# Senpai-sama06/real-time-audio-visual-zooming

Measured on AMD Instinct MI355X. Metric: beamformed TF-bins/sec (2-ch, 1024-pt STFT) + SIR dB delta vs reference, higher is better.
Workload: dtype f32; 1 GPU; configs[1]: B=256 utterances/GPU, 2 interferers, oracle IBM, 1024-pt STFT hop 512 @16 kHz, 4.0 s utterances; batch_per_gpu=256, global_batch=256, samples=64000, n_fft=1024, hop=512, parallelism=utterance-sharded x1, RCCL metric all-reduce only, input_batches=2, tf_bins_per_utt=64638, mask=ibm, postfilter=ibm, normalize=peak

## Files before the change

real-time-audio-visual-zooming_amd/csrc/avz_chain_exact.hpp:

```cpp
#pragma once
#include "avz_chain_common.hpp"
#include "avz_ibm_exact.hpp"

namespace avz {
__device__ __forceinline__ int pick(uint32_t packed, int i) {
  return (int)(signed char)(packed >> (8 * i));
}
template <int N>
struct XLds {
  using C = KCfg<N>;
  using X = XGeo<N>;
  static constexpr int FR = 4;
  static constexpr int MP = N / 2 + 4;
  static constexpr int MIC_BYTES = FR / C::FPW * C::WAVE_BYTES;
  static constexpr int MAG_OFF = (4 * X::SCRATCH > MIC_BYTES) ? 4 * X::SCRATCH : MIC_BYTES;
  static constexpr int TWL_OFF = MAG_OFF + 2 * FR * MP * 4;
  static constexpr int WIN_OFF = TWL_OFF + (N / 2) * 16;
  static constexpr int SLOT_OFF = WIN_OFF + N * 4;
  static constexpr int SCAN_OFF = SLOT_OFF + FR * 32;
  static constexpr int SCAN_INTS = 256;
  static constexpr int WL = 32;
  static constexpr int WL_OFF = SCAN_OFF + 256 * 4;
  static constexpr int CTL_OFF = WL_OFF + WL * 16;
  static constexpr int END = CTL_OFF + 32;
  static_assert(C::FPW == 2 && END <= CGeo<N>::SLOT_LDS, "exact phase LDS");
};

struct XSlot {
  int unit, f, e, b, L, c, flags, pad;
};
__device__ __forceinline__ XSlot slot_u(const XSlot* sl, int g) {
  const XSlot v = sl[g];
  XSlot s;
  s.unit = __builtin_amdgcn_readfirstlane(v.unit);
  s.f = __builtin_amdgcn_readfirstlane(v.f);
  s.e = 0;
  s.b = __builtin_amdgcn_readfirstlane(v.b);
  s.L = __builtin_amdgcn_readfirstlane(v.L);
  s.c = __builtin_amdgcn_readfirstlane(v.c);
  s.flags = __builtin_amdgcn_readfirstlane(v.flags);
  s.pad = 0;
  return s;
}

template <int N, bool PER_BIN>
__device__ __forceinline__ void exact_round(KArgs& A, unsigned char* lds, const XSlot* sl, int ns,
                                            Acc32 (&pacc)[CGeo<N>::BPT + 1],
                                            uint32_t (&pbits)[CGeo<N>::BPT + 1]) {
  using C = KCfg<N>;
  using G = CGeo<N>;
  using X = XGeo<N>;
  using XL = XLds<N>;
  constexpr int NT = G::NT, H = G::H, F = G::F, BPT = G::BPT, PPL = C::PPL, MP = XL::MP;
  const int tid = threadIdx.x, lane = tid & 63;
  const int wave = __builtin_amdgcn_readfirstlane(tid >> 6);
  float* const mag = reinterpret_cast<float*>(lds + XL::MAG_OFF);
  const cd* const twl = reinterpret_cast<const cd*>(lds + XL::TWL_OFF);
  const float* const win = reinterpret_cast<const float*>(lds + XL::WIN_OFF);
  cd* const buf = reinterpret_cast<cd*>(lds + wave * X::SCRATCH);
  AVZ_STAMP_DECL();
  AVZ_STAMP_INIT();
  AVZ_XT_LAP_BEGIN(xr_prev);
  int lane_o = lane;
  opaque_i(lane_o);
  const int ga = wave >> 1, gb = (wave >> 1) + 2;
  const float* const refp = (wave & 1) ? A.ref_int : A.ref_tgt;
  float xa[N / 64], xb[N / 64];
  if (ga < ns) {
    const XSlot s = slot_u(sl, ga);
    ref_frame_load<N>(make_rsrc(refp + (long long)s.b * A.ref_stride, s.L),
                      (s.c * kChunk + s.f) * H - N / 2, lane_o, xa);
  }
  if (gb < ns) {
    const XSlot s = slot_u(sl, gb);
    ref_frame_load<N>(make_rsrc(refp + (long long)s.b * A.ref_stride, s.L),
                      (s.c * kChunk + s.f) * H - N / 2, lane_o, xb);
  }
  if (ga < ns) ref_spectrum_exact<N>(xa, twl, win, buf, mag + (2 * ga + (wave & 1)) * MP, lane_o);
  AVZ_STAMP(4);
  AVZ_XT_LAP(8, xr_prev);
  cf v[PPL];
  LaneMap<N> lm;
  lm.init(lane_o);
  const int gm = C::FPW * wave + lm.grp;
  if (wave < XL::FR / C::FPW) {
    const XSlot s = slot_u(sl, 0);
    const float* mixb = A.mix + (long long)s.b * A.mix_stride;
    const rsrc_t r_m0 = make_rsrc(mixb, s.L), r_m1 = make_rsrc(mixb + A.ch_stride, s.L);
    const bool on = gm < ns;
    const int fm = sl[on ? gm : 0].f;
    const int s0 = (s.c * kChunk + fm) * H - N / 2 + lm.in0;
#pragma unroll
    for (int r = 0; r < PPL; ++r) {
      v[r].x = on ? bload(r_m0, s0 + C::IN_STRIDE * r) : 0.0f;
      v[r].y = on ? bload(r_m1, s0 + C::IN_STRIDE * r) : 0.0f;
    }
  }
  if (gb < ns) {
    int lane_b = lane;
    opaque_i(lane_b);
    ref_spectrum_exact<N>(xb, twl, win, buf, mag + (2 * gb + (wave & 1)) * MP, lane_b);
  }
  AVZ_STAMP(5);
  lds_barrier();
  AVZ_STAMP(6);
  AVZ_XT_LAP(9, xr_prev);
  if (wave < XL::FR / C::FPW) {
    WinCoef<N> wc;
    wc.init(lm);
    cf* const spec = slot_ptr<N>(lds, gm);
    if constexpr (N == 1024) {
      Fft1024x2 f;
      f.l = lm.out0;
      window_apply(v, wc.a0, wc.ac, wc.as);
      f.forward(v, spec, reinterpret_cast<const cf*>(lds + G::TW_OFF));
      static_for<0, 32>([&](auto k) { spec[lm.out0 + 32 * k] = v[k]; });
    } else {
      Fft512x2 f;
      f.init(lane_o);
      window_fft<N>(v, wc, f, spec, lm);
    }
  }
  AVZ_STAMP(7);
  lds_barrier();
  AVZ_STAMP(8);
  AVZ_XT_LAP(10, xr_prev);
  unsigned long long n_exact = 0;
  for (int g = 0; g < ns; ++g) {
    const XSlot s = slot_u(sl, g);
    const cf* Zm = slot_ptr<N>(lds, g);
    auto put = [&](int j, int k, const Acc32& a, bool dfr, bool noise) {
      if (dfr) {
        pacc[j].c00 += a.c00;
        pacc[j].c11 += a.c11;
        pacc[j].c01r += a.c01r;
        pacc[j].c01i += a.c01i;
        pacc[j].cm += a.cm;
        pbits[j] |= (noise ? 1u : 0u) << s.f;
      }
    };
#pragma unroll
    for (int j = 0; j < BPT; ++j) {
      const int kb = tid + j * NT;
      const int kp = (N - kb) & (N - 1);
      const bool dfr =
          PER_BIN ? ((A.xdfr[(long long)s.unit * F + kb] >> s.f) & 1u)
                  : ((s.flags & 1) &&
                     ((A.xunc[((long long)s.unit * kChunk + s.f) * 32 + (kb & 31)] >> (kb >> 5)) & 1u));
      Acc32 a;
      a.zero();
      bool noise = false;
      if (dfr) {
        noise = mag[(2 * g + 1) * MP + kb] > mag[(2 * g) * MP + kb];
        cf x0, x1;
        split_pair2(Zm[kb], Zm[kp], x0, x1);
        a.add_sel(x0, x1, noise);
        a.cm = noise ? 1.0f : 0.0f;
        n_exact += 1;
      }
      put(j, kb, a, dfr, noise);
    }
    if (tid == NT - 1) {
      const bool dfr = (s.flags >> 1) & 1;
      Acc32 a;
      a.zero();
      bool noise = false;
      if (dfr) {
        noise = mag[(2 * g + 1) * MP + N / 2] > mag[(2 * g) * MP + N / 2];
        cf y0, y1;
        split_pair2(Zm[N / 2], Zm[N / 2], y0, y1);
        const float wn = noise ? 1.0f : 0.0f;
        a.add(y0, y1, wn, wn);
        n_exact += 1;
      }
      put(BPT, N / 2, a, dfr, noise);
    }
  }
  if (A.xstat && n_exact) atomicAdd(A.xstat + 1, n_exact);
  AVZ_STAMP(9);
  lds_barrier();
  AVZ_STAMP(10);
  AVZ_XT_LAP(11, xr_prev);
}

constexpr int kSparseMax = 12;

constexpr uint32_t kXOpen = 0x80000000u;
constexpr int kXRound = 2;
struct XPieces {
  uint32_t sp;
  int n_sp, nr, npr, n;
};
__device__ __forceinline__ XPieces x_pieces(uint32_t pend, uint32_t big) {
  XPieces q;
  q.sp = pend & ~big;
  q.n_sp = q.sp ? 1 : 0;
  q.nr = (__popc(big) + kXRound - 1) / kXRound;
  q.npr = min(q.nr, kXPieces - q.n_sp);
  q.n = q.n_sp + q.npr;
  return q;
}
__device__ __forceinline__ bool x_has_piece(uint32_t v) {
  return (v & kXOpen) && (v & 0xffffu) < ((v >> 16) & 0xffu);
}

template <int N>
__device__ __forceinline__ void exact_sparse(KArgs& A, unsigned char* lds, int b, int L, int c,
                                             const int* items, int n,
                                             Acc32 (&pacc)[CGeo<N>::BPT + 1],
                                             uint32_t (&pbits)[CGeo<N>::BPT + 1]) {
  using G = CGeo<N>;
  using XL = XLds<N>;
  constexpr int H = N / 2, NT = G::NT, BPT = G::BPT;
  const int tid = threadIdx.x, lane = tid & 63;
  const int wave = __builtin_amdgcn_readfirstlane(tid >> 6);
  const cd* const twl = reinterpret_cast<const cd*>(lds + XL::TWL_OFF);
  const float* const win = reinterpret_cast<const float*>(lds + XL::WIN_OFF);
  float* const res = reinterpret_cast<float*>(lds);
  const rsrc_t rt = make_rsrc(A.ref_tgt + (long long)b * A.ref_stride, L);
  const rsrc_t ri = make_rsrc(A.ref_int + (long long)b * A.ref_stride, L);
  const float* mixb = A.mix + (long long)b * A.mix_stride;
  const rsrc_t rm0 = make_rsrc(mixb, L), rm1 = make_rsrc(mixb + A.ch_stride, L);
  for (int it = wave; it < n; it += NT / 64) {
    const int item = __builtin_amdgcn_readfirstlane(items[it]);
    const int f = item >> 16, k = item & 0xffff;
    const int s0 = (c * kChunk + f) * H - N / 2;
    float st[N / 64], si[N / 64], sm0[N / 64], sm1[N / 64];
#pragma unroll
    for (int r = 0; r < N / 64; ++r) {
      const int m = lane + 64 * r;
      st[r] = bload(rt, s0 + m);
      si[r] = bload(ri, s0 + m);
      sm0[r] = bload(rm0, s0 + m);
      sm1[r] = bload(rm1, s0 + m);
    }
    double tr = 0.0, ti = 0.0, ir = 0.0, ii = 0.0, ac = 0.0, bs = 0.0, as = 0.0, bc = 0.0;
#pragma unroll
    for (int r = 0; r < N / 64; ++r) {
      const int m = lane + 64 * r;
      const double w = (double)win[m];
      const double xt = w * (double)st[r], xi = w * (double)si[r];
      const double a = w * (double)sm0[r], bb = w * (double)sm1[r];
      const cd tw = xtw_at<N>(twl, (k * m) & (N - 1));
      tr = fma(xt, tw.x, tr);
      ti = fma(xt, tw.y, ti);
      ir = fma(xi, tw.x, ir);
      ii = fma(xi, tw.y, ii);
      ac = fma(a, tw.x, ac);
      bs = fma(bb, tw.y, bs);
      as = fma(a, tw.y, as);
      bc = fma(bb, tw.x, bc);
    }
#pragma unroll
    for (int o = 32; o > 0; o >>= 1) {
      tr += __shfl_xor(tr, o, 64);
      ti += __shfl_xor(ti, o, 64);
      ir += __shfl_xor(ir, o, 64);
      ii += __shfl_xor(ii, o, 64);
      ac += __shfl_xor(ac, o, 64);
      bs += __shfl_xor(bs, o, 64);
      as += __shfl_xor(as, o, 64);
      bc += __shfl_xor(bc, o, 64);
    }
    if (lane == 0) {
      const bool noise = np_abs_c64((float)ir, (float)ii) > np_abs_c64((float)tr, (float)ti);
      constexpr double sc = 2.0 / N;
      const cf zk = {(float)(sc * (ac - bs)), (float)(sc * (as + bc))};
      const cf zp = {(float)(sc * (ac + bs)), (float)(sc * (bc - as))};
      Acc32 t;
      t.zero();
      cf x0, x1;
      split_pair2(zk, zp, x0, x1);
      if (k == N / 2) {
        const float wn = noise ? 1.0f : 0.0f;
        t.add(x0, x1, wn, wn);
      } else {
        t.add_sel(x0, x1, noise);
        t.cm = noise ? 1.0f : 0.0f;
      }
      float* q = res + 6 * it;
      q[0] = noise ? 1.0f : 0.0f;
      q[1] = t.c00;
      q[2] = t.c11;
      q[3] = t.c01r;
      q[4] = t.c01i;
      q[5] = t.cm;
    }
  }
  __syncthreads();
  for (int it = 0; it < n; ++it) {
    const int item = items[it];
    const int f = item >> 16, k = item & 0xffff;
    const int j = k == N / 2 ? BPT : k / NT;
    if (k == N / 2 ? tid == NT - 1 : (k % NT) == tid) {
      const float* q = res + 6 * it;
#pragma unroll
      for (int jj = 0; jj <= BPT; ++jj) {
        if (jj != j) continue;
        pacc[jj].c00 += q[1];
        pacc[jj].c11 += q[2];
        pacc[jj].c01r += q[3];
        pacc[jj].c01i += q[4];
        pacc[jj].cm += q[5];
        pbits[jj] |= (q[0] != 0.0f ? 1u : 0u) << f;
      }
    }
  }
  if (A.xstat && tid == 0) atomicAdd(A.xstat + 1, (unsigned long long)n);
  __syncthreads();
}

template <int N, bool PER_BIN, class CA>
__device__ __forceinline__ void exact_set_slot(CA& A, XSlot* sl, int g, int u, int f, int gx,
                                               int n_items, int n_whole, int P) {
  constexpr int F = N / 2 + 1;
  XSlot s;
  s.unit = u;
  s.f = f;
  s.e = -1;
  unit_item<F>(A, u, gx, n_items, n_whole, P, s.b, s.c);
  s.L = utt_len(A, s.b);
  const uint4 r = reinterpret_cast<const uint4*>(A.xpend)[u];
  s.flags = (PER_BIN ? 0 : (int)((r.y >> f) & 1u)) | (int)(((r.z >> f) & 1u) << 1);
  s.pad = 0;
  sl[g] = s;
}

template <int N, bool PER_BIN>
__device__ __forceinline__ void exact_unit(KArgs& A, unsigned char* lds, int u, int gx, int n_items,
                                           int n_whole, int P) {
  using G = CGeo<N>;
  using XL = XLds<N>;
  constexpr int F = N / 2 + 1, NT = G::NT, BPT = G::BPT, FR = XL::FR;
  const int tid = threadIdx.x;
  XSlot* const sl = reinterpret_cast<XSlot*>(lds + XL::SLOT_OFF);
  const uint4 rec = reinterpret_cast<const uint4*>(A.xpend)[u];
  const uint32_t pend = rec.x;
  if (pend == 0u || rec.w != 0u) return;
  int b, c;
  float* const Pt = unit_item<F>(A, u, gx, n_items, n_whole, P, b, c);
  if (A.xstat && tid == 0) atomicAdd(A.xstat, (unsigned long long)__popc(pend));
  Acc32 pacc[BPT + 1];
  uint32_t pbits[BPT + 1];
#pragma unroll
  for (int j = 0; j <= BPT; ++j) {
    const int kk = j < BPT ? tid + j * NT : N / 2;
    pbits[j] = 0u;
    if (j < BPT || tid == NT - 1) {
      pacc[j].c00 = Pt[0 * F + kk];
      pacc[j].c11 = Pt[1 * F + kk];
      pacc[j].c01r = Pt[2 * F + kk];
      pacc[j].c01i = Pt[3 * F + kk];
      pacc[j].cm = Pt[4 * F + kk];
    } else {
      pacc[j].zero();
    }
  }
  uint32_t rest = pend;
  if constexpr (!PER_BIN) {
    int* const items = reinterpret_cast<int*>(lds + XL::SCAN_OFF);
    int* const ctl = reinterpret_cast<int*>(lds + XL::CTL_OFF);
    uint32_t* const wsm = reinterpret_cast<uint32_t*>(lds + 16384);
    const uint32_t has_words = reinterpret_cast<const uint4*>(A.xpend)[u].y;
#pragma unroll
    for (int i = 0; i < kChunk / (G::NT / 32); ++i) {
      const int f = (tid >> 5) + (G::NT / 32) * i;
      if ((pend >> f) & 1u)
        wsm[f * 32 + (tid & 31)] =
            ((has_words >> f) & 1u) ? A.xunc[((long long)u * kChunk + f) * 32 + (tid & 31)] : 0u;
    }
    __syncthreads();
    if (tid < 64) {
      const uint32_t nyq = reinterpret_cast<const uint4*>(A.xpend)[u].z;
      int base = 0;
      uint32_t sparse = 0u;
      for (uint32_t todo = pend; todo != 0u; todo &= todo - 1u) {
        const int f = __builtin_ctz(todo);
        const uint32_t w = tid < 32 ? wsm[f * 32 + tid] : 0u;
        int inc = __popc(w);
#pragma unroll
        for (int o = 1; o < 32; o <<= 1) {
          const int y = __shfl_up(inc, o, 64);
          if ((tid & 63) >= o) inc += y;
        }
        const int tot = __shfl(inc, 31, 64), ny = (nyq >> f) & 1u;
        if (tot + ny <= kSparseMax && base + tot + ny <= XL::SCAN_INTS) {
          int at = base + inc - __popc(w);
          for (uint32_t x = w; x != 0u; x &= x - 1u) items[at++] = (f << 16) | (tid + 32 * __builtin_ctz(x));
          if (ny && tid == 0) items[base + tot] = (f << 16) | (N / 2);
          base += tot + ny;
          sparse |= 1u << f;
        }
      }
      if (tid == 0) {
        ctl[0] = base;
        ctl[1] = (int)sparse;
      }
    }
    __syncthreads();
    const int n_sp = ctl[0];
    rest &= ~(uint32_t)ctl[1];
    if (n_sp > 0) exact_sparse<N>(A, lds, b, utt_len(A, b), c, items, n_sp, pacc, pbits);
  }
  while (rest != 0u) {
    if (tid < FR) {
      uint32_t x = rest;
      for (int i = 0; i < tid && x; ++i) x &= x - 1u;
      if (x) exact_set_slot<N, PER_BIN>(A, sl, tid, u, __builtin_ctz(x), gx, n_items, n_whole, P);
    }
    const int ns = min(FR, __popc(rest));
    for (int i = 0; i < ns; ++i) rest &= rest - 1u;
    __syncthreads();
    exact_round<N, PER_BIN>(A, lds, sl, ns, pacc, pbits);
  }
  uint32_t* const MW = A.mwords + ((long long)b * A.nchunk + c) * F;
#pragma unroll
  for (int j = 0; j <= BPT; ++j) {
    const int kk = j < BPT ? tid + j * NT : N / 2;
    if (j < BPT || tid == NT - 1) {
      Pt[0 * F + kk] = pacc[j].c00;
      Pt[1 * F + kk] = pacc[j].c11;
      Pt[2 * F + kk] = pacc[j].c01r;
      Pt[3 * F + kk] = pacc[j].c01i;
      Pt[4 * F + kk] = pacc[j].cm;
      if (pbits[j]) atomicOr(MW + kk, pbits[j]);
    }
  }
}

template <int N>
__device__ __forceinline__ void exact_sparse_frames(KArgs& A, unsigned char* lds, int u, int b,
                                                    int c, uint32_t frames,
                                                    Acc32 (&pacc)[CGeo<N>::BPT + 1],
                                                    uint32_t (&pbits)[CGeo<N>::BPT + 1]) {
  using G = CGeo<N>;
  using XL = XLds<N>;
  const int tid = threadIdx.x;
  int* const items = reinterpret_cast<int*>(lds + XL::SCAN_OFF);
  int* const ctl = reinterpret_cast<int*>(lds + XL::CTL_OFF);
  uint32_t* const wsm = reinterpret_cast<uint32_t*>(lds + 16384);
  const uint4 rec = reinterpret_cast<const uint4*>(A.xpend)[u];
#pragma unroll
  for (int i = 0; i < kChunk / (G::NT / 32); ++i) {
    const int f = (tid >> 5) + (G::NT / 32) * i;
    if ((frames >> f) & 1u)
      wsm[f * 32 + (tid & 31)] =
          ((rec.y >> f) & 1u) ? A.xunc[((long long)u * kChunk + f) * 32 + (tid & 31)] : 0u;
  }
  __syncthreads();
  uint32_t todo = frames;
  while (todo != 0u) {
    if (tid < 64) {
      int base = 0;
      uint32_t took = 0u;
      for (uint32_t t = todo; t != 0u; t &= t - 1u) {
        const int f = __builtin_ctz(t);
        const uint32_t w = tid < 32 ? wsm[f * 32 + tid] : 0u;
        int inc = __popc(w);
#pragma unroll
        for (int o = 1; o < 32; o <<= 1) {
          const int y = __shfl_up(inc, o, 64);
          if ((tid & 63) >= o) inc += y;
        }
        const int tot = __shfl(inc, 31, 64), ny = (rec.z >> f) & 1u;
        if (base + tot + ny > XL::SCAN_INTS) break;
        int at = base + inc - __popc(w);
        for (uint32_t x = w; x != 0u; x &= x - 1u) items[at++] = (f << 16) | (tid + 32 * __builtin_ctz(x));
        if (ny && tid == 0) items[base + tot] = (f << 16) | (N / 2);
        base += tot + ny;
        took |= 1u << f;
      }
      if (tid == 0) {
        ctl[0] = base;
        ctl[1] = (int)took;
      }
    }
    __syncthreads();
    const int n = ctl[0];
    todo &= ~(uint32_t)ctl[1];
    exact_sparse<N>(A, lds, b, utt_len(A, b), c, items, n, pacc, pbits);
  }
}

template <int N, bool PER_BIN>
__device__ __forceinline__ void exact_piece(KArgs& A, unsigned char* lds, int u, int p, int gx,
                                            int n_items, int n_whole, int P) {
  using G = CGeo<N>;
  using XL = XLds<N>;
  constexpr int F = N / 2 + 1, NT = G::NT, BPT = G::BPT, FR = XL::FR;
  const int tid = threadIdx.x;
  XSlot* const sl = reinterpret_cast<XSlot*>(lds + XL::SLOT_OFF);
  int* const ctl = reinterpret_cast<int*>(lds + XL::CTL_OFF);
  const uint4 rec = reinterpret_cast<const uint4*>(A.xpend)[u];
  const XPieces q = x_pieces(rec.x, rec.w);
  int b, c;
  float* const Pt = unit_item<F>(A, u, gx, n_items, n_whole, P, b, c);
  Acc32 pacc[BPT + 1];
  uint32_t pbits[BPT + 1];
#pragma unroll
  for (int j = 0; j <= BPT; ++j) {
    pacc[j].zero();
    pbits[j] = 0u;
  }
  if (p < q.n_sp) {
    if (A.xstat && tid == 0) atomicAdd(A.xstat, (unsigned long long)__popc(q.sp));
    if constexpr (!PER_BIN) exact_sparse_frames<N>(A, lds, u, b, c, q.sp, pacc, pbits);
  } else {
    constexpr int R = kXRound;
    static_assert(R <= FR, "round frames");
    const int g = p - q.n_sp, r0 = g * q.nr / q.npr, r1 = (g + 1) * q.nr / q.npr;
    if (A.xstat && tid == 0)
      atomicAdd(A.xstat, (unsigned long long)(min(R * r1, __popc(rec.w)) - R * r0));
    const int L = utt_len(A, b);
    uint32_t rest = rec.w;
    for (int i = 0; i < r0 * R; ++i) rest &= rest - 1u;
    for (int r = r0; r < r1; ++r) {
      if (tid < R) {
        uint32_t x = rest;
        for (int i = 0; i < tid && x; ++i) x &= x - 1u;
        if (x) {
          const int f = __builtin_ctz(x);
          XSlot s;
          s.unit = u;
          s.f = f;
          s.e = -1;
          s.b = b;
          s.L = L;
          s.c = c;
          s.flags = (PER_BIN ? 0 : (int)((rec.y >> f) & 1u)) | (int)(((rec.z >> f) & 1u) << 1);
          s.pad = 0;
          sl[tid] = s;
        }
      }
      const int ns = min(R, __popc(rest));
      for (int i = 0; i < ns; ++i) rest &= rest - 1u;
      __syncthreads();
      exact_round<N, PER_BIN>(A, lds, sl, ns, pacc, pbits);
    }
  }
  uint32_t* const MW = A.mwords + ((long long)b * A.nchunk + c) * F;
  float* const R = A.xres + ((long long)u * kXPieces + p) * 5 * F;
#pragma unroll
  for (int j = 0; j <= BPT; ++j) {
    const int kk = j < BPT ? tid + j * NT : N / 2;
    if (j < BPT || tid == NT - 1) {
      if (pbits[j]) atomicOr(MW + kk, pbits[j]);
      if (q.n == 1) {
        Pt[0 * F + kk] = Pt[0 * F + kk] + pacc[j].c00;
        Pt[1 * F + kk] = Pt[1 * F + kk] + pacc[j].c11;
        Pt[2 * F + kk] = Pt[2 * F + kk] + pacc[j].c01r;
        Pt[3 * F + kk] = Pt[3 * F + kk] + pacc[j].c01i;
        Pt[4 * F + kk] = Pt[4 * F + kk] + pacc[j].cm;
      } else {
        R[0 * F + kk] = pacc[j].c00;
        R[1 * F + kk] = pacc[j].c11;
        R[2 * F + kk] = pacc[j].c01r;
        R[3 * F + kk] = pacc[j].c01i;
        R[4 * F + kk] = pacc[j].cm;
      }
    }
  }
#ifdef AVZ_XTRACE
  const unsigned long long tf = __builtin_amdgcn_s_memrealtime();
#endif
  __syncthreads();
  if (tid == 0) {
    bool last = true;
    if (q.n > 1) {
      __builtin_amdgcn_fence(__ATOMIC_RELEASE, "agent");
      const uint32_t arrived =
          __hip_atomic_fetch_add(A.xst + 2 * u + 1, 1u, __ATOMIC_RELAXED, __HIP_MEMORY_SCOPE_AGENT) + 1u;
      last = arrived == (uint32_t)q.n;
      if (last) __builtin_amdgcn_fence(__ATOMIC_ACQUIRE, "agent");
    }
    ctl[4] = last ? 1 : 0;
  }
  __syncthreads();
#ifdef AVZ_XTRACE
  const unsigned long long tm = __builtin_amdgcn_s_memrealtime();
  if (tid == 0 && g_stamps) g_stamps[blockIdx.x * 16 + 6] += tm - tf;
#endif
  if (ctl[4]) {
    if (q.n > 1) {
      const float* const R0 = A.xres + (long long)u * kXPieces * 5 * F;
      constexpr int M = (5 * F + NT - 1) / NT;
      float v[M];
#pragma unroll
      for (int m = 0; m < M; ++m) v[m] = tid + m * NT < 5 * F ? Pt[tid + m * NT] : 0.0f;
      for (int pp = 0; pp < q.n; ++pp) {
        float t[M];
#pragma unroll
        for (int m = 0; m < M; ++m)
          t[m] = tid + m * NT < 5 * F ? R0[(long long)pp * 5 * F + tid + m * NT] : 0.0f;
#pragma unroll
        for (int m = 0; m < M; ++m) v[m] += t[m];
      }
#pragma unroll
      for (int m = 0; m < M; ++m)
        if (tid + m * NT < 5 * F) Pt[tid + m * NT] = v[m];
    }
    if (tid == 0) {
      __hip_atomic_store(A.xst + 2 * u + 1, 0u, __ATOMIC_RELAXED, __HIP_MEMORY_SCOPE_AGENT);
      __hip_atomic_store(A.xst + 2 * u, 0u, __ATOMIC_RELAXED, __HIP_MEMORY_SCOPE_AGENT);
      __hip_atomic_fetch_and(A.xhint + (u >> 5), ~(1u << (u & 31)), __ATOMIC_RELAXED,
                             __HIP_MEMORY_SCOPE_AGENT);
    }
  }
  __syncthreads();
#ifdef AVZ_XTRACE
  if (tid == 0 && g_stamps) g_stamps[blockIdx.x * 16 + 7] += __builtin_amdgcn_s_memrealtime() - tm;
#endif
}

__device__ __forceinline__ int exact_claim(KArgs& A, int n_units, int* cand) {
  const int lane = threadIdx.x & 63;
  const int nw = (n_units + 31) >> 5;
  const int w_start = (int)(((long long)blockIdx.x * nw) / gridDim.x);
  for (;;) {
    int count = 0;
    for (int w0 = 0; w0 < nw && count < 64; w0 += 64) {
      const int wi = w0 + lane;
      int wid = w_start + wi;
      if (wid >= nw) wid -= nw;
      const uint32_t bits =
          wi < nw ? __hip_atomic_load(A.xhint + wid, __ATOMIC_RELAXED, __HIP_MEMORY_SCOPE_AGENT) : 0u;
      const int cnt = __popc(bits);
      int pre = cnt;
#pragma unroll
      for (int o = 1; o < 64; o <<= 1) {
        const int y = __shfl_up(pre, o, 64);
        if (lane >= o) pre += y;
      }
      const int tot = __shfl(pre, 63, 64);
      int pos = count + pre - cnt;
      for (uint32_t x = bits; x != 0u && pos < 64; x &= x - 1u) cand[pos++] = wid * 32 + __builtin_ctz(x);
      count += tot;
    }
    count = min(count, 64);
    if (count == 0) return -1;
    __builtin_amdgcn_fence(__ATOMIC_RELEASE, "wavefront");
    __builtin_amdgcn_wave_barrier();
    __builtin_amdgcn_fence(__ATOMIC_ACQUIRE, "wavefront");
    const int uid = lane < count ? cand[lane] : -1;
    const uint32_t v =
        uid >= 0 ? __hip_atomic_load(A.xst + 2 * uid, __ATOMIC_RELAXED, __HIP_MEMORY_SCOPE_AGENT) : 0u;
    const unsigned long long m = __ballot(x_has_piece(v));
    if (m == 0ull) return -1;
    int k = (int)(blockIdx.x % (unsigned)__popcll(m));
    unsigned long long mm = m;
    for (; k > 0; --k) mm &= mm - 1ull;
    const int src = __builtin_ctzll(mm);
    int res = -1;
    if (lane == src) {
      const uint32_t old =
          __hip_atomic_fetch_add(A.xst + 2 * uid, 1u, __ATOMIC_RELAXED, __HIP_MEMORY_SCOPE_AGENT);
      if (x_has_piece(old)) {
        __builtin_amdgcn_fence(__ATOMIC_ACQUIRE, "agent");
        res = (uid << 8) | (int)(old & 0xffu);
      }
    }
    res = __shfl(res, src, 64);
    if (res >= 0) return res;
    __builtin_amdgcn_wave_barrier();
  }
}

template <int N, int MASK, bool IRM, bool SPLIT, class TW>
__device__ __forceinline__ void ibm_exact_units(unsigned char* lds, int gx, int n_items) {
  KArgs& A = kernarg_chain_args();
  using G = CGeo<N>;
  using XL = XLds<N>;
  constexpr bool SHARE = N == 1024 && !std::is_same<TW, NoTw>::value;
  constexpr bool PER_BIN = !(N == 1024 && !IRM && SHARE);
  AVZ_XT(1, __builtin_amdgcn_s_memrealtime());
  if (A.ibm_cert <= 0.0f) return;
  const int tid = threadIdx.x;
  const int P = SPLIT && A.a_pieces > 1 ? A.a_pieces : 1;
  const int n_whole = P > 1 ? A.a_whole : n_items;
  __syncthreads();
  const uint32_t mine = *reinterpret_cast<const uint32_t*>(lds + G::MISC_OFF + 56);
  auto tables = [&]() {
    int t = threadIdx.x;
    opaque_i(t);
    xtab_fill<N>(A.xtw, A.xwin, reinterpret_cast<cd*>(lds + XL::TWL_OFF),
                 reinterpret_cast<float*>(lds + XL::WIN_OFF), t, G::NT);
    __syncthreads();
  };
  bool have_tables = false;
  int seq = 0;
  auto one = [&](int u) {
    const int k = seq++;
    if (!((mine >> min(k, 31)) & 1u)) return;
    const uint4 rec = reinterpret_cast<const uint4*>(A.xpend)[u];
    if (rec.x == 0u || rec.w != 0u) return;
    if (k >= 31) {
      int b, c;
      unit_item<G::F>(A, u, gx, n_items, n_whole, P, b, c);
      const int L = utt_len(A, b);
      if (L < N || c >= ((L + G::H - 1) / G::H + 1 + kChunk - 1) / kChunk) return;
    }
    if (!have_tables) {
      tables();
      have_tables = true;
    }
    exact_unit<N, PER_BIN>(A, lds, u, gx, n_items, n_whole, P);
  };
  const int n_end = n_whole + (n_items - n_whole) * P;
  for (int u = blockIdx.x; u < n_end; u += gridDim.x) one(u < n_whole ? u : n_items + u - n_whole);
  AVZ_XT(2, __builtin_amdgcn_s_memrealtime());
  {
    const int n_units = n_items + (n_end - n_whole);
    int* const ctl = reinterpret_cast<int*>(lds + XLds<N>::CTL_OFF);
    for (;;) {
      AVZ_XT_BEGIN(tc);
      if (tid < 64) {
        const int got = exact_claim(A, n_units, reinterpret_cast<int*>(lds + XLds<N>::SCAN_OFF));
        if (tid == 0) ctl[2] = got;
      }
      AVZ_XT_END(14, tc);
      __syncthreads();
      const int got = ctl[2];
      __syncthreads();
      if (got < 0) break;
      if (!have_tables) {
        AVZ_XT_BEGIN(tt);
        tables();
        have_tables = true;
        AVZ_XT_END(15, tt);
      }
      AVZ_XT_BEGIN(t0x);
      exact_piece<N, PER_BIN>(A, lds, got >> 8, got & 0xff, gx, n_items, n_whole, P);
#ifdef AVZ_XTRACE
      if (tid == 0 && g_stamps) {
        unsigned long long* st = g_stamps + blockIdx.x * 16;
        st[4] += 1;
        st[5] += __builtin_amdgcn_s_memrealtime() - t0x;
      }
#endif
    }
  }
  AVZ_XT(3, __builtin_amdgcn_s_memrealtime());
}
}
```

Baseline: 77.71 billion TF-bins/s.

## Compute only the louder reference spectrum with a bound-based fallback for the quiet one

Each wave now handles one slot. It computes the windowed L1 norm of both reference frames and runs the FFT only on the louder one, using the quieter frame's norm as a magnitude upper bound tau. If the loud magnitude exceeds tau for every deferred bin, the noise decision is settled and the second FFT is skipped. Otherwise a fallback pass computes the quiet spectrum. The change also prefetches the deferred-bin mask words up front, overlaps the mic FFT with the reference work when there are two or fewer slots, and unrolls the cross-piece reduction loads so they are issued together. Costs are extra double-precision norm work, an additional barrier and atomicOr, more register pressure, and a divergent fallback path.

```diff
diff --git a/real-time-audio-visual-zooming_amd/csrc/avz_chain_exact.hpp b/real-time-audio-visual-zooming_amd/csrc/avz_chain_exact.hpp
--- a/real-time-audio-visual-zooming_amd/csrc/avz_chain_exact.hpp
+++ b/real-time-audio-visual-zooming_amd/csrc/avz_chain_exact.hpp
@@ -22,8 +22,10 @@
   static constexpr int WL = 32;
   static constexpr int WL_OFF = SCAN_OFF + 256 * 4;
   static constexpr int CTL_OFF = WL_OFF + WL * 16;
-  static constexpr int END = CTL_OFF + 32;
+  static constexpr int BND_OFF = CTL_OFF + 32;
+  static constexpr int END = BND_OFF + 48;
   static_assert(C::FPW == 2 && END <= CGeo<N>::SLOT_LDS, "exact phase LDS");
+  static_assert(2 * X::SCRATCH <= C::WAVE_BYTES && 2 * C::WAVE_BYTES <= MAG_OFF, "pair round LDS");
 };
 
 struct XSlot {
@@ -58,32 +60,75 @@
   const cd* const twl = reinterpret_cast<const cd*>(lds + XL::TWL_OFF);
   const float* const win = reinterpret_cast<const float*>(lds + XL::WIN_OFF);
   cd* const buf = reinterpret_cast<cd*>(lds + wave * X::SCRATCH);
+  int* const bnd = reinterpret_cast<int*>(lds + XL::BND_OFF);
+  const bool pair = ns <= 2;
   AVZ_STAMP_DECL();
   AVZ_STAMP_INIT();
   AVZ_XT_LAP_BEGIN(xr_prev);
   int lane_o = lane;
   opaque_i(lane_o);
-  const int ga = wave >> 1, gb = (wave >> 1) + 2;
-  const float* const refp = (wave & 1) ? A.ref_int : A.ref_tgt;
-  float xa[N / 64], xb[N / 64];
-  if (ga < ns) {
-    const XSlot s = slot_u(sl, ga);
-    ref_frame_load<N>(make_rsrc(refp + (long long)s.b * A.ref_stride, s.L),
-                      (s.c * kChunk + s.f) * H - N / 2, lane_o, xa);
-  }
-  if (gb < ns) {
-    const XSlot s = slot_u(sl, gb);
-    ref_frame_load<N>(make_rsrc(refp + (long long)s.b * A.ref_stride, s.L),
-                      (s.c * kChunk + s.f) * H - N / 2, lane_o, xb);
-  }
-  if (ga < ns) ref_spectrum_exact<N>(xa, twl, win, buf, mag + (2 * ga + (wave & 1)) * MP, lane_o);
+  if (tid == 0) bnd[8] = 0;
+  uint32_t dw[XL::FR][BPT];
+#pragma unroll
+  for (int g = 0; g < XL::FR; ++g) {
+    const bool on = g < ns;
+    const XSlot s = slot_u(sl, on ? g : 0);
+#pragma unroll
+    for (int j = 0; j < BPT; ++j) {
+      const int kb = tid + j * NT;
+      if constexpr (PER_BIN) {
+        dw[g][j] = on ? A.xdfr[(long long)s.unit * F + kb] : 0u;
+      } else {
+        dw[g][j] = (on && (s.flags & 1))
+                       ? A.xunc[((long long)s.unit * kChunk + s.f) * 32 + (kb & 31)]
+                       : 0u;
+      }
+    }
+  }
+  const bool own = wave < ns;
+  if (own) {
+    const XSlot s = slot_u(sl, wave);
+    const int s0 = (s.c * kChunk + s.f) * H - N / 2;
+    float xt[N / 64], xi[N / 64];
+    ref_frame_load<N>(make_rsrc(A.ref_tgt + (long long)s.b * A.ref_stride, s.L), s0, lane_o, xt);
+    ref_frame_load<N>(make_rsrc(A.ref_int + (long long)s.b * A.ref_stride, s.L), s0, lane_o, xi);
+    double st = 0.0, si = 0.0;
+#pragma unroll
+    for (int r = 0; r < X::RX; ++r) {
+      const float2 w = reinterpret_cast<const float2*>(win)[lane_o + 64 * r];
+      st += fabs((double)w.x * (double)xt[2 * r]) + fabs((double)w.y * (double)xt[2 * r + 1]);
+      si += fabs((double)w.x * (double)xi[2 * r]) + fabs((double)w.y * (double)xi[2 * r + 1]);
+    }
+#pragma unroll
+    for (int o = 32; o > 0; o >>= 1) {
+      st += __shfl_xor(st, o, 64);
+      si += __shfl_xor(si, o, 64);
+    }
+    const int loud = __builtin_amdgcn_readfirstlane(si > st ? 1 : 0);
+    const double sq = loud ? st : si;
+    float tau = __builtin_inff();
+    if (sq == 0.0 || sq >= 0x1p-100) {
+      const double t = sq * (1.0 + 0x1p-20);
+      tau = (float)t;
+      if ((double)tau < t) tau = __uint_as_float(__float_as_uint(tau) + 1u);
+    }
+    if (lane == 0) {
+      bnd[2 * wave] = loud;
+      bnd[2 * wave + 1] = (int)__float_as_uint(tau);
+    }
+    float xl[N / 64];
+#pragma unroll
+    for (int r = 0; r < N / 64; ++r) xl[r] = loud ? xi[r] : xt[r];
+    ref_spectrum_exact<N>(xl, twl, win, buf, mag + (2 * wave + loud) * MP, lane_o);
+  }
   AVZ_STAMP(4);
-  AVZ_XT_LAP(8, xr_prev);
   cf v[PPL];
   LaneMap<N> lm;
   lm.init(lane_o);
-  const int gm = C::FPW * wave + lm.grp;
-  if (wave < XL::FR / C::FPW) {
+  const int gm = C::FPW * (pair ? 0 : wave) + lm.grp;
+  cf* const spec = slot_ptr<N>(lds, pair ? 2 + lm.grp : gm);
+  const bool mic_wave = pair ? wave == 2 : wave < XL::FR / C::FPW;
+  if (mic_wave) {
     const XSlot s = slot_u(sl, 0);
     const float* mixb = A.mix + (long long)s.b * A.mix_stride;
     const rsrc_t r_m0 = make_rsrc(mixb, s.L), r_m1 = make_rsrc(mixb + A.ch_stride, s.L);
@@ -96,19 +141,9 @@
       v[r].y = on ? bload(r_m1, s0 + C::IN_STRIDE * r) : 0.0f;
     }
   }
-  if (gb < ns) {
-    int lane_b = lane;
-    opaque_i(lane_b);
-    ref_spectrum_exact<N>(xb, twl, win, buf, mag + (2 * gb + (wave & 1)) * MP, lane_b);
-  }
-  AVZ_STAMP(5);
-  lds_barrier();
-  AVZ_STAMP(6);
-  AVZ_XT_LAP(9, xr_prev);
-  if (wave < XL::FR / C::FPW) {
+  auto mic_fft = [&]() {
     WinCoef<N> wc;
     wc.init(lm);
-    cf* const spec = slot_ptr<N>(lds, gm);
     if constexpr (N == 1024) {
       Fft1024x2 f;
       f.l = lm.out0;
@@ -120,15 +155,68 @@
       f.init(lane_o);
       window_fft<N>(v, wc, f, spec, lm);
     }
-  }
-  AVZ_STAMP(7);
+  };
+  if (pair && mic_wave) mic_fft();
+  AVZ_XT_LAP(8, xr_prev);
+  AVZ_STAMP(5);
   lds_barrier();
+  AVZ_STAMP(6);
+  uint32_t dmask = 0u, und = 0u;
+#pragma unroll
+  for (int g = 0; g < XL::FR; ++g) {
+    if (g < ns) {
+      const XSlot s = slot_u(sl, g);
+      const float* const ml = mag + (2 * g + bnd[2 * g]) * MP;
+      const float tau = __uint_as_float((uint32_t)bnd[2 * g + 1]);
+#pragma unroll
+      for (int j = 0; j < BPT; ++j) {
+        const int kb = tid + j * NT;
+        const bool dfr = PER_BIN ? ((dw[g][j] >> s.f) & 1u) : ((dw[g][j] >> (kb >> 5)) & 1u);
+        if (dfr) {
+          dmask |= 1u << (g * (BPT + 1) + j);
+          if (!(ml[kb] > tau)) und |= 1u << g;
+        }
+      }
+      if (tid == NT - 1 && ((s.flags >> 1) & 1)) {
+        dmask |= 1u << (g * (BPT + 1) + BPT);
+        if (!(ml[N / 2] > tau)) und |= 1u << g;
+      }
+    }
+  }
+  if (und) atomicOr(reinterpret_cast<unsigned int*>(bnd + 8), und);
+  lds_barrier();
+  const uint32_t fb = (uint32_t)__builtin_amdgcn_readfirstlane(bnd[8]);
+  if (fb) {
+    if (own && ((fb >> wave) & 1u)) {
+      const XSlot s = slot_u(sl, wave);
+      const int quiet = 1 - __builtin_amdgcn_readfirstlane(bnd[2 * wave]);
+      float xq[N / 64];
+      int lane_b = lane;
+      opaque_i(lane_b);
+      ref_frame_load<N>(make_rsrc((quiet ? A.ref_int : A.ref_tgt) + (long long)s.b * A.ref_stride, s.L),
+                        (s.c * kChunk + s.f) * H - N / 2, lane_b, xq);
+      ref_spectrum_exact<N>(xq, twl, win, buf, mag + (2 * wave + quiet) * MP, lane_b);
+    }
+    lds_barrier();
+  }
+  AVZ_XT_LAP(9, xr_prev);
+  if (!pair) {
+    if (mic_wave) mic_fft();
+    AVZ_STAMP(7);
+    lds_barrier();
+  }
   AVZ_STAMP(8);
   AVZ_XT_LAP(10, xr_prev);
   unsigned long long n_exact = 0;
   for (int g = 0; g < ns; ++g) {
     const XSlot s = slot_u(sl, g);
-    const cf* Zm = slot_ptr<N>(lds, g);
+    const cf* Zm = slot_ptr<N>(lds, pair ? g + 2 : g);
+    const int loud = bnd[2 * g];
+    const float* const ml = mag + (2 * g + loud) * MP;
+    const float tau = __uint_as_float((uint32_t)bnd[2 * g + 1]);
+    auto decide = [&](int k) {
+      return ml[k] > tau ? loud != 0 : mag[(2 * g + 1) * MP + k] > mag[(2 * g) * MP + k];
+    };
     auto put = [&](int j, int k, const Acc32& a, bool dfr, bool noise) {
       if (dfr) {
         pacc[j].c00 += a.c00;
@@ -143,15 +231,12 @@
     for (int j = 0; j < BPT; ++j) {
       const int kb = tid + j * NT;
       const int kp = (N - kb) & (N - 1);
-      const bool dfr =
-          PER_BIN ? ((A.xdfr[(long long)s.unit * F + kb] >> s.f) & 1u)
-                  : ((s.flags & 1) &&
-                     ((A.xunc[((long long)s.unit * kChunk + s.f) * 32 + (kb & 31)] >> (kb >> 5)) & 1u));
+      const bool dfr = (dmask >> (g * (BPT + 1) + j)) & 1u;
       Acc32 a;
       a.zero();
       bool noise = false;
       if (dfr) {
-        noise = mag[(2 * g + 1) * MP + kb] > mag[(2 * g) * MP + kb];
+        noise = decide(kb);
         cf x0, x1;
         split_pair2(Zm[kb], Zm[kp], x0, x1);
         a.add_sel(x0, x1, noise);
@@ -166,7 +251,7 @@
       a.zero();
       bool noise = false;
       if (dfr) {
-        noise = mag[(2 * g + 1) * MP + N / 2] > mag[(2 * g) * MP + N / 2];
+        noise = decide(N / 2);
         cf y0, y1;
         split_pair2(Zm[N / 2], Zm[N / 2], y0, y1);
         const float wn = noise ? 1.0f : 0.0f;
@@ -587,13 +672,21 @@
       float v[M];
 #pragma unroll
       for (int m = 0; m < M; ++m) v[m] = tid + m * NT < 5 * F ? Pt[tid + m * NT] : 0.0f;
-      for (int pp = 0; pp < q.n; ++pp) {
-        float t[M];
-#pragma unroll
-        for (int m = 0; m < M; ++m)
-          t[m] = tid + m * NT < 5 * F ? R0[(long long)pp * 5 * F + tid + m * NT] : 0.0f;
-#pragma unroll
-        for (int m = 0; m < M; ++m) v[m] += t[m];
+      float t[kXPieces][M];
+#pragma unroll
+      for (int pp = 0; pp < kXPieces; ++pp) {
+        if (pp < q.n) {
+#pragma unroll
+          for (int m = 0; m < M; ++m)
+            t[pp][m] = tid + m * NT < 5 * F ? R0[(long long)pp * 5 * F + tid + m * NT] : 0.0f;
+        }
+      }
+#pragma unroll
+      for (int pp = 0; pp < kXPieces; ++pp) {
+        if (pp < q.n) {
+#pragma unroll
+          for (int m = 0; m < M; ++m) v[m] += t[pp][m];
+        }
       }
 #pragma unroll
       for (int m = 0; m < M; ++m)
```

New measurement: 78.29 billion TF-bins/s (median of 6 runs). Within noise of the previous version (+0.7%).
